# Arsham-001/tsu-emulator

Measured on AMD Instinct MI355X. Metric: spin-updates/sec on L×L 2D Ising Gibbs sweep; achieved HBM GB/s vs peak, higher is better.
Workload: dtype int8

## Files before the change

### tsu-emulator_amd/csrc/ising2d_tiled.hip

```cpp
#include "ising2d.h"

#include <type_traits>
#include <vector>

typedef short v2s __attribute__((ext_vector_type(2)));
typedef unsigned short v2us __attribute__((ext_vector_type(2)));

struct TiledParams {
    const int8_t* src;
    int8_t* dst;
    long long pitch;
    int rows, nchunks;
    int cols;
    int q_shift;
    int tile_h;
    int flex_ty;
    int r_begin, r_end;
    long long row0, total_rows;
    int wrap_rows, ghost;
    int k;
    int tiles_x;
    int ty_first, ty_stride;
    uint32_t k0, k1, sweep0, tag_hi, tag_lo;
    uint32_t tblH0, tblH1, tblL0, tblL1;
    uint32_t t3H0, t3H1, t3L0, t3L1;
    int open;
    uint64_t thr[25];
};

static __host__ __device__ __forceinline__ void tile_rows(const TiledParams& p, int ty, int& row_off, int& H) {
    H = p.tile_h;
    row_off = ty * p.tile_h;
    if (p.flex_ty > 0) {
        const long long half = (p.r_end - p.r_begin + 1) / 2;
        row_off = 2 * (int)(ty * half / p.flex_ty);
        H = 2 * (int)((ty + 1) * half / p.flex_ty) - row_off;
    }
}
static __host__ __device__ __forceinline__ bool tile_holds_wrap(const TiledParams& p, int ty, int k, long long& rg0) {
    int H, row_off;
    tile_rows(p, ty, row_off, H);
    rg0 = p.row0 + p.r_begin + row_off - 2 * k;
    if (p.open) return false;
    rg0 %= p.total_rows;
    if (rg0 < 0) rg0 += p.total_rows;
    return rg0 + H + 4 * k > p.total_rows;
}
static __host__ __device__ __forceinline__ bool wrap_by_mask(const TiledParams& p) { return (p.total_rows & (p.total_rows - 1)) == 0; }

static __device__ __forceinline__ uint32_t perm(uint32_t s0, uint32_t s1, uint32_t sel) {
    return __builtin_amdgcn_perm(s0, s1, sel);
}
static __device__ __forceinline__ uint32_t subsat16(uint32_t a, uint32_t b) {
    return __builtin_bit_cast(uint32_t, __builtin_elementwise_sub_sat(__builtin_bit_cast(v2s, a), __builtin_bit_cast(v2s, b)));
}
static __device__ __forceinline__ uint32_t minu16(uint32_t a, uint32_t b) {
    return __builtin_bit_cast(uint32_t, __builtin_elementwise_min(__builtin_bit_cast(v2us, a), __builtin_bit_cast(v2us, b)));
}

static __device__ __noinline__ u32x4 resolve_ties(u32x4 d, u32x4 w, uint32_t cnt_lo, uint32_t cnt_hi, const uint64_t* s_thr,
                                                  uint32_t cq, uint32_t Rg, uint32_t hs, uint32_t tag_lo, uint32_t k0,
                                                  uint32_t k1, uint32_t edge = 0) {
    const u32x4 l = tsu_philox(cq, Rg, hs, tag_lo, k0, k1);
#define TSU_FIX(DW, WW, LW, CNT, B0, M0)                                                                        \
    _Pragma("unroll") for (int hlf = 0; hlf < 2; ++hlf) {                                                       \
        const uint32_t sh = 16u * hlf;                                                                          \
        if (((DW >> sh) & 0xFFFFu) == 0) {                                                                      \
            const uint32_t c = (CNT >> (8 * (B0 + hlf))) & 0xFFu;                                               \
            const uint32_t m = M0 + hlf;                                                                        \
            const uint32_t deg = 4u - (edge & 1u) - ((m == 0 && (edge & 2u)) ? 1u : 0u) - ((m == (edge >> 4) && (edge & 4u)) ? 1u : 0u); \
            const uint64_t u = ((uint64_t)(((WW >> sh) & 0xFFFFu) ^ 0x8000u) << 16) | ((LW >> sh) & 0xFFFFu);   \
            const uint32_t f = (u < s_thr[deg * 5 + c]) ? 0x8000u : 0x0001u;       \
            DW = (DW & ~(0xFFFFu << sh)) | (f << sh);                                                           \
        }                                                                                                       \
    }
    TSU_FIX(d.x, w.x, l.x, cnt_lo, 0, 0)
    TSU_FIX(d.y, w.y, l.y, cnt_lo, 2, 2)
    TSU_FIX(d.z, w.z, l.z, cnt_hi, 0, 4)
    TSU_FIX(d.w, w.w, l.w, cnt_hi, 2, 6)
#undef TSU_FIX
    return d;
}

struct PhiloxKeys {
    uint32_t a[10], b[10];
};

static __device__ __forceinline__ PhiloxKeys make_keys(uint32_t k0, uint32_t k1) {
    PhiloxKeys K;
#pragma unroll
    for (int r = 0; r < 10; ++r) {
        uint32_t x = k0 + (uint32_t)r * TSU_PHILOX_W0, y = k1 + (uint32_t)r * TSU_PHILOX_W1;
        if (r > 0) asm volatile("v_mov_b32 %0, %1" : "=v"(x) : "s"(x));
        asm volatile("v_mov_b32 %0, %1" : "=v"(y) : "s"(y));
        K.a[r] = x;
        K.b[r] = y;
    }
    return K;
}

static __device__ __forceinline__ uint32_t and_xor(uint32_t a, uint32_t b, uint32_t c) { return __builtin_amdgcn_bitop3_b32(a, b, c, 0x6A); }

static __device__ __forceinline__ uint32_t philox_y0(uint32_t hs, uint32_t k0) {
    uint32_t y = (uint32_t)(((uint64_t)TSU_PHILOX_M1 * hs) >> 32) ^ k0;
    asm volatile("v_mov_b32 %0, %1" : "=v"(y) : "s"(y));
    return y;
}

static __device__ __forceinline__ u32x4 philox_vk(uint32_t c0, uint32_t row, uint32_t rmask, uint32_t y0, uint32_t c2, uint32_t c3,
                                                  const PhiloxKeys& K) {
    uint32_t c1;
    {
        const uint64_t p0 = (uint64_t)TSU_PHILOX_M0 * c0;
        const uint64_t p1 = (uint64_t)TSU_PHILOX_M1 * c2;
        const uint32_t n0 = and_xor(row, rmask, y0);
        const uint32_t n2 = tsu_xor3((uint32_t)(p0 >> 32), c3, K.b[0]);
        c1 = (uint32_t)p1;
        c3 = (uint32_t)p0;
        c0 = n0;
        c2 = n2;
    }
#pragma unroll
    for (int r = 1; r < 10; ++r) {
        uint64_t p0 = (uint64_t)TSU_PHILOX_M0 * c0;
        uint64_t p1 = (uint64_t)TSU_PHILOX_M1 * c2;
        uint32_t n0 = tsu_xor3((uint32_t)(p1 >> 32), c1, K.a[r]);
        uint32_t n2 = tsu_xor3((uint32_t)(p0 >> 32), c3, K.b[r]);
        c1 = (uint32_t)p1;
        c3 = (uint32_t)p0;
        c0 = n0;
        c2 = n2;
    }
    return u32x4{c0, c1, c2, c3};
}

struct Rows2Ctx {
    const uint64_t* s_thr;
    int total_rows;
    int rg_tile0, wrap_tr;
    uint32_t rmask;
    uint32_t tag_hi, tag_lo, k0, k1;
    uint32_t tblH0, tblH1, tblL0, tblL1;
    uint32_t t3H0, t3H1, t3L0, t3L1;
    int last_row;
    bool lft, rgt;
    uint32_t r_par, r_slot;
    uint32_t rm_lo, rm_hi;
    uint64_t vm_e, vm_o;
    uint32_t nvm_e, nvm_o;
    int sh_next, sh_prev;
};

static __device__ __forceinline__ u32x4 compare_octet(const u32x4& w, uint32_t cnt_lo, uint32_t cnt_hi, uint32_t tH0,
                                                      uint32_t tH1, uint32_t tL0, uint32_t tL1) {
    const uint32_t Hl = perm(tH1, tH0, cnt_lo), Ll = perm(tL1, tL0, cnt_lo);
    const uint32_t Hh = perm(tH1, tH0, cnt_hi), Lh = perm(tL1, tL0, cnt_hi);
    u32x4 d;
    d.x = subsat16(w.x, perm(Hl, Ll, 0x05010400u));
    d.y = subsat16(w.y, perm(Hl, Ll, 0x07030602u));
    d.z = subsat16(w.z, perm(Hh, Lh, 0x05010400u));
    d.w = subsat16(w.w, perm(Hh, Lh, 0x07030602u));
    return d;
}

static __device__ __forceinline__ u32x4 compare_octet_open(const u32x4& w, uint32_t cnt_lo, uint32_t cnt_hi, const Rows2Ctx& c,
                                                           bool row_edge, bool l0, bool r7) {
    uint32_t Hl = perm(c.tblH1, c.tblH0, cnt_lo), Ll = perm(c.tblL1, c.tblL0, cnt_lo);
    uint32_t Hh = perm(c.tblH1, c.tblH0, cnt_hi), Lh = perm(c.tblL1, c.tblL0, cnt_hi);
    if (row_edge | l0 | r7) {
        const uint32_t rl = r7 ? c.rm_lo : 0u, rh = r7 ? c.rm_hi : 0u;
        const uint32_t il = cnt_lo + ((row_edge && l0) ? 0x00000004u : 0u) + (row_edge ? (rl & 0x04040404u) : 0u);
        const uint32_t ih = cnt_hi + (row_edge ? (rh & 0x04040404u) : 0u);
        const uint32_t ml = row_edge ? 0xFFFFFFFFu : ((l0 ? 0x000000FFu : 0u) | rl), mh = row_edge ? 0xFFFFFFFFu : rh;
        Hl = (Hl & ~ml) | (perm(c.t3H1, c.t3H0, il) & ml);
        Ll = (Ll & ~ml) | (perm(c.t3L1, c.t3L0, il) & ml);
        Hh = (Hh & ~mh) | (perm(c.t3H1, c.t3H0, ih) & mh);
        Lh = (Lh & ~mh) | (perm(c.t3L1, c.t3L0, ih) & mh);
    }
    u32x4 d;
    d.x = subsat16(w.x, perm(Hl, Ll, 0x05010400u));
    d.y = subsat16(w.y, perm(Hl, Ll, 0x07030602u));
    d.z = subsat16(w.z, perm(Hh, Lh, 0x05010400u));
    d.w = subsat16(w.w, perm(Hh, Lh, 0x07030602u));
    return d;
}

static __device__ __forceinline__ bool has_zero_field(const u32x4& d) {
    const uint32_t mn = minu16(minu16(d.x, d.y), minu16(d.z, d.w));
    return ((mn & 0xFFFFu) == 0) | ((mn >> 16) == 0);
}

static __device__ __forceinline__ uint64_t pack_flags(const u32x4& d) {
    const uint32_t nlo = perm(d.y, d.x, 0x0B0A0908u) & 0x01010101u;
    const uint32_t nhi = perm(d.w, d.z, 0x0B0A0908u) & 0x01010101u;
    return (uint64_t)nlo | ((uint64_t)nhi << 32);
}

template <int NO>
static __device__ __forceinline__ void edge_rows(const Rows2Ctx& c, int to_wrap, int tr, int& rga, int& rgb) {
    constexpr int SPAN = 2 * ((NO - 1 + 63) / NO) + 1;
    const int s_off = to_wrap > 0 ? c.rg_tile0 : c.rg_tile0 - c.total_rows;
    rga = tr + s_off;
    rgb = rga + 1;
    if (__builtin_expect((uint32_t)(to_wrap - 1) < (uint32_t)SPAN, 0)) {
        rga = tr + c.rg_tile0;
        asm volatile("" : "+v"(rga));
        rgb = rga + 1;
        if (rga >= c.total_rows) rga -= c.total_rows;
        if (rgb >= c.total_rows) rgb -= c.total_rows;
    }
}

#define TSU_LDS __attribute__((address_space(3)))
static __device__ __forceinline__ uint32_t lds_addr(const void* p) { return (uint32_t)(uintptr_t)(const TSU_LDS char*)p; }
template <typename T>
static __device__ __forceinline__ T lds_ld(uint32_t a) { return *(const TSU_LDS T*)(uintptr_t)a; }
template <typename T>
static __device__ __forceinline__ void lds_st(uint32_t a, T v) { *(TSU_LDS T*)(uintptr_t)a = v; }

template <typename E, int NO>
struct TilePlanes {
    E* base;
// ... 17 lines not shown
    const u32x4 w0 = philox_vk(cq, (uint32_t)rga, c.rmask, y0, hs, c.tag_hi, K);
    const u32x4 w1 = philox_vk(cq, (uint32_t)rgb, c.rmask, y0, hs, c.tag_hi, K);
    __builtin_amdgcn_sched_barrier(0);
    const uint32_t C0l = (uint32_t)R1, C0h = (uint32_t)(R1 >> 32), C1l = (uint32_t)R2, C1h = (uint32_t)(R2 >> 32);
    uint32_t S0l = P0 ? __builtin_amdgcn_alignbyte(C0h, C0l, 1) : __builtin_amdgcn_alignbyte(C0l, A0, 3);
    uint32_t S0h = P0 ? __builtin_amdgcn_alignbyte(A0, C0h, 1) : __builtin_amdgcn_alignbyte(C0h, C0l, 3);
    uint32_t S1l = P0 ? __builtin_amdgcn_alignbyte(C1l, A1, 3) : __builtin_amdgcn_alignbyte(C1h, C1l, 1);
    uint32_t S1h = P0 ? __builtin_amdgcn_alignbyte(C1h, C1l, 3) : __builtin_amdgcn_alignbyte(A1, C1h, 1);
    if (SEAM) {
        const uint64_t nxa = (Na & 0xFFull) << c.sh_next, pva = (Na >> c.sh_prev) & 0xFFull;
        const uint64_t nxb = (Nb & 0xFFull) << c.sh_next, pvb = (Nb >> c.sh_prev) & 0xFFull;
        const uint64_t Sa = P0 ? ((R1 >> 8) | nxa) : ((R1 << 8) | pva);
        const uint64_t Sb = P0 ? ((R2 << 8) | pvb) : ((R2 >> 8) | nxb);
        S0l = (uint32_t)Sa; S0h = (uint32_t)(Sa >> 32);
        S1l = (uint32_t)Sb; S1h = (uint32_t)(Sb >> 32);
    }
    const uint32_t ml = C0l + C1l, mh = C0h + C1h;
    const uint32_t cnt0l = (uint32_t)R0 + ml + S0l, cnt0h = (uint32_t)(R0 >> 32) + mh + S0h;
    const uint32_t cnt1l = (uint32_t)R3 + ml + S1l, cnt1h = (uint32_t)(R3 >> 32) + mh + S1h;
    u32x4 d0, d1;
    uint32_t edge_a = 0, edge_b = 0;
    if (OPEN) {
        const bool ea = rga == 0 || rga == c.last_row, eb = rgb == 0 || rgb == c.last_row;
        const bool la = !P0 && c.lft, ra = c.rgt && c.r_par == (uint32_t)P0, lb = P0 && c.lft, rb = c.rgt && c.r_par != (uint32_t)P0;
        d0 = compare_octet_open(w0, cnt0l, cnt0h, c, ea, la, ra);
        d1 = compare_octet_open(w1, cnt1l, cnt1h, c, eb, lb, rb);
        edge_a = (ea ? 1u : 0u) | (la ? 2u : 0u) | (ra ? 4u : 0u) | (c.r_slot << 4);
        edge_b = (eb ? 1u : 0u) | (lb ? 2u : 0u) | (rb ? 4u : 0u) | (c.r_slot << 4);
    } else {
        d0 = compare_octet(w0, cnt0l, cnt0h, c.tblH0, c.tblH1, c.tblL0, c.tblL1);
        d1 = compare_octet(w1, cnt1l, cnt1h, c.tblH0, c.tblH1, c.tblL0, c.tblL1);
    }
    const uint32_t mn = minu16(minu16(minu16(d0.x, d0.y), minu16(d0.z, d0.w)), minu16(minu16(d1.x, d1.y), minu16(d1.z, d1.w)));
    if (__builtin_expect(((mn & 0xFFFFu) == 0) | ((mn >> 16) == 0), 0)) {
        if (has_zero_field(d0)) d0 = resolve_ties(d0, w0, cnt0l, cnt0h, c.s_thr, cq, (uint32_t)rga & c.rmask, hs, c.tag_lo, c.k0, c.k1, edge_a);
        if (has_zero_field(d1)) d1 = resolve_ties(d1, w1, cnt1l, cnt1h, c.s_thr, cq, (uint32_t)rgb & c.rmask, hs, c.tag_lo, c.k0, c.k1, edge_b);
    }
    uint64_t n0 = pack_flags(d0), n1 = pack_flags(d1);
    if (OPEN) {
        n0 = (rga < 0 || rga > c.last_row) ? 0 : (n0 & (P0 ? c.vm_o : c.vm_e));
        n1 = (rgb < 0 || rgb > c.last_row) ? 0 : (n1 & (P0 ? c.vm_e : c.vm_o));
    }
    if (SEAM) {
        n0 &= c.vm_e;
        n1 &= c.vm_e;
    }
    lds_st<uint64_t>(a + RS + DO, n0);
    lds_st<uint64_t>(a + 2 * RS + DO, n1);
}

template <int NO, int RL, int KAPPA, int P0, bool EDGE, bool OPEN, bool SEAM = false>
static __device__ __forceinline__ void sweep_pairs(const Rows2Ctx& c, const PhiloxKeys& K, uint32_t hs, uint32_t y0, uint32_t a, int rg, int n, bool tail,
                                                   uint32_t cq) {
    int to_wrap = EDGE ? c.wrap_tr - __builtin_amdgcn_readfirstlane(rg) : 0;
    bool live = true;
#pragma unroll 1
    for (int i = n; i >= 0; --i) {
        if (i == 0) live = tail;
        asm volatile("" : "+v"(a), "+v"(rg));
        if (live) pair_step<NO, KAPPA, P0, EDGE, OPEN, SEAM>(c, K, hs, y0, a, rg, to_wrap, cq);
        a += 2 * RL * 2 * NO * 8;
        rg += 2 * RL;
        to_wrap -= 2 * RL;
    }
}


static __device__ __forceinline__ uint32_t nib_shift_next(uint32_t X, uint32_t N) {
    const uint32_t hi = (N << 4) | __builtin_amdgcn_ubfe(X, 4u, 4u);
// ... 22 lines not shown
    constexpr int DO = (KAPPA ? NO : -NO) * 4;
    const uint32_t R0 = lds_ld<uint32_t>(a), R1 = lds_ld<uint32_t>(a + RS);
    const uint32_t R2 = lds_ld<uint32_t>(a + 2 * RS), R3 = lds_ld<uint32_t>(a + 3 * RS);
    const uint32_t A0 = lds_ld<uint32_t>(a + RS + (P0 ? 4 : -4));
    const uint32_t A1 = lds_ld<uint32_t>(a + 2 * RS + (P0 ? -4 : 4));
    __builtin_amdgcn_sched_barrier(0);
    int rga = rg, rgb = rg + 1;
    if (EDGE) edge_rows<NO>(c, to_wrap, rg, rga, rgb);
    const u32x4 w0 = philox_vk(cq, (uint32_t)rga, c.rmask, y0, hs, c.tag_hi, K);
    const u32x4 w1 = philox_vk(cq, (uint32_t)rgb, c.rmask, y0, hs, c.tag_hi, K);
    __builtin_amdgcn_sched_barrier(0);
    const uint32_t Sa = SEAM ? (P0 ? nib_shift_next_seam(R1, A0, c.sh_next) : nib_shift_prev_seam(R1, A0, c.sh_prev))
                             : (P0 ? nib_shift_next(R1, A0) : nib_shift_prev(R1, A0));
    const uint32_t Sb = SEAM ? (P0 ? nib_shift_prev_seam(R2, A1, c.sh_prev) : nib_shift_next_seam(R2, A1, c.sh_next))
                             : (P0 ? nib_shift_prev(R2, A1) : nib_shift_next(R2, A1));
    const uint32_t mid = R1 + R2;
    const uint32_t cnt0 = R0 + mid + Sa, cnt1 = R3 + mid + Sb;
    const uint32_t cnt0l = cnt0 & 0x0F0F0F0Fu, cnt0h = (cnt0 >> 4) & 0x0F0F0F0Fu;
    const uint32_t cnt1l = cnt1 & 0x0F0F0F0Fu, cnt1h = (cnt1 >> 4) & 0x0F0F0F0Fu;
    u32x4 d0, d1;
    uint32_t edge_a = 0, edge_b = 0;
    if (OPEN) {
        const bool ea = rga == 0 || rga == c.last_row, eb = rgb == 0 || rgb == c.last_row;
        const bool la = !P0 && c.lft, ra = c.rgt && c.r_par == (uint32_t)P0, lb = P0 && c.lft, rb = c.rgt && c.r_par != (uint32_t)P0;
        d0 = compare_octet_open(w0, cnt0l, cnt0h, c, ea, la, ra);
        d1 = compare_octet_open(w1, cnt1l, cnt1h, c, eb, lb, rb);
        edge_a = (ea ? 1u : 0u) | (la ? 2u : 0u) | (ra ? 4u : 0u) | (c.r_slot << 4);
        edge_b = (eb ? 1u : 0u) | (lb ? 2u : 0u) | (rb ? 4u : 0u) | (c.r_slot << 4);
    } else {
        d0 = compare_octet(w0, cnt0l, cnt0h, c.tblH0, c.tblH1, c.tblL0, c.tblL1);
        d1 = compare_octet(w1, cnt1l, cnt1h, c.tblH0, c.tblH1, c.tblL0, c.tblL1);
    }
    const uint32_t mn = minu16(minu16(minu16(d0.x, d0.y), minu16(d0.z, d0.w)), minu16(minu16(d1.x, d1.y), minu16(d1.z, d1.w)));
    if (__builtin_expect(((mn & 0xFFFFu) == 0) | ((mn >> 16) == 0), 0)) {
        if (has_zero_field(d0)) d0 = resolve_ties(d0, w0, cnt0l, cnt0h, c.s_thr, cq, (uint32_t)rga & c.rmask, hs, c.tag_lo, c.k0, c.k1, edge_a);
        if (has_zero_field(d1)) d1 = resolve_ties(d1, w1, cnt1l, cnt1h, c.s_thr, cq, (uint32_t)rgb & c.rmask, hs, c.tag_lo, c.k0, c.k1, edge_b);
    }
    uint32_t n0 = nib_pack(d0), n1 = nib_pack(d1);
    if (OPEN) {
        n0 = (rga < 0 || rga > c.last_row) ? 0u : (n0 & (P0 ? c.nvm_o : c.nvm_e));
        n1 = (rgb < 0 || rgb > c.last_row) ? 0u : (n1 & (P0 ? c.nvm_e : c.nvm_o));
    }
    if (SEAM) {
        n0 &= c.nvm_e;
        n1 &= c.nvm_e;
    }
    lds_st<uint32_t>(a + RS + DO, n0);
    lds_st<uint32_t>(a + 2 * RS + DO, n1);
}

template <int NO, int RL, int KAPPA, int P0, bool EDGE, bool OPEN = false, bool SEAM = false>
static __device__ __forceinline__ void sweep_pairs_nib(const Rows2Ctx& c, const PhiloxKeys& K, uint32_t hs, uint32_t y0, uint32_t a, int rg, int n, bool tail,
                                                       uint32_t cq) {
    int to_wrap = EDGE ? c.wrap_tr - __builtin_amdgcn_readfirstlane(rg) : 0;
    bool live = true;
#pragma unroll 1
    for (int i = n; i >= 0; --i) {
        if (i == 0) live = tail;
        asm volatile("" : "+v"(a), "+v"(rg));
        if (live) pair_step_nib<NO, KAPPA, P0, EDGE, OPEN, SEAM>(c, K, hs, y0, a, rg, to_wrap, cq);
        a += 2 * RL * 2 * NO * 4;
        rg += 2 * RL;
        to_wrap -= 2 * RL;
    }
}

template <int NO, int RL, int KAPPA, int P0, bool EDGE, bool OPEN, bool SEAM, bool NIB>
static __device__ __forceinline__ void half_sweep(const Rows2Ctx& c, const PhiloxKeys& K, int TR, uint32_t sweep, int s, uint32_t a_thr, int al,
                                                  uint32_t cq) {
// ... 25 lines not shown
                                                        int al, uint32_t cq) {
#pragma unroll 1
    for (int s = 0; s < kg; ++s) {
        half_sweep<NO, RL, 0, P0, EDGE, OPEN, SEAM, NIB>(c, K, TR, sweep_g + (uint32_t)s, s, a_thr, al, cq);
        half_sweep<NO, RL, 1, P0, EDGE, OPEN, SEAM, NIB>(c, K, TR, sweep_g + (uint32_t)s, s, a_thr, al, cq);
    }
}

static __device__ __forceinline__ void xst(uint64_t* p, uint64_t v) { __hip_atomic_store(p, v, __ATOMIC_RELAXED, __HIP_MEMORY_SCOPE_AGENT); }
static __device__ __forceinline__ uint64_t xld(const uint64_t* p) { return __hip_atomic_load(p, __ATOMIC_RELAXED, __HIP_MEMORY_SCOPE_AGENT); }

struct ResidentParams {
    uint64_t* xbuf;
    uint32_t gen0;
    int* err;
    int n_gen, k_last, tiles_y;
    int wrap_y;
    int wrap_x;
    long long* dbg;
};

template <int HT, int WO, int THREADS, bool OPEN = false, bool RESIDENT = false, bool NIB = false>
static __device__ __forceinline__ void tile_body(const TiledParams& p, const int8_t* __restrict__ src, int8_t* __restrict__ dst,
                                                 const int k, const uint32_t sweep0, const int tx, const int ty, uint64_t* lds,
                                                 const PhiloxKeys& K, const ResidentParams* R = nullptr) {
    constexpr int NO = WO + 2;
    constexpr int RLMAX = THREADS / NO;
    int H, row_off;
    tile_rows(p, ty, row_off, H);
    const int TR = H + 4 * k;
    constexpr int RL = RLMAX;
    using E = typename std::conditional<NIB, uint32_t, uint64_t>::type;
    const TilePlanes<E, NO> P{reinterpret_cast<E*>(lds + 1)};
    uint64_t* s_thr = reinterpret_cast<uint64_t*>((reinterpret_cast<uintptr_t>(P.base + 2 * TR * NO + NO + 1) + 7u) & ~(uintptr_t)7u);
    const int tid = threadIdx.x;
    if (tid < 25) s_thr[tid] = p.thr[tid];

    const int q0 = tx * WO + p.q_shift, r0 = p.r_begin + row_off, Rb = r0 - 2 * k;

    const int al = tid / NO, oct = tid - al * NO;
    int cqi = q0 - 1 + oct;
    const bool col_out = OPEN && (cqi < 0 || cqi >= p.nchunks);
    if (!OPEN) {
        if (cqi < 0) cqi += p.nchunks;
        if (cqi >= p.nchunks) cqi -= p.nchunks;
        if (cqi >= p.nchunks) cqi -= p.nchunks;
    }
    const uint32_t cq = (uint32_t)cqi;
    int nv = p.cols - 16 * cqi;
    if (col_out) nv = 0;
    if (nv > 16) nv = 16;
    auto first_sites = [](int n) { return n >= 8 ? 0x0101010101010101ull : (((1ull << (8 * n)) - 1) & 0x0101010101010101ull); };
    const uint64_t vm_e = first_sites((nv + 1) >> 1), vm_o = first_sites(nv >> 1);

    if (al < RLMAX) {
        const int8_t* col = src + 16 * (long long)(OPEN ? (cqi < 0 ? 0 : (cqi >= p.nchunks ? p.nchunks - 1 : cqi)) : cqi);
        constexpr int LB = 4;
        for (int tr0 = al; tr0 < TR; tr0 += LB * RLMAX) {
            uint4 v[LB];
#pragma unroll
            for (int b = 0; b < LB; ++b) {
                const int tr = tr0 + b * RLMAX;
                const int rl = Rb + (tr < TR ? tr : TR - 1);
                int srow;
                if (p.wrap_rows) srow = rl < 0 ? rl + p.rows : (rl >= p.rows ? rl - p.rows : rl);
                else srow = rl < -p.ghost ? -p.ghost : (rl >= p.rows + p.ghost ? p.rows + p.ghost - 1 : rl);
                v[b] = *reinterpret_cast<const uint4*>(col + (long long)srow * p.pitch);
            }
#pragma unroll
            for (int b = 0; b < LB; ++b) {
                const int tr = tr0 + b * RLMAX;
                if (tr < TR) {
                    const uint32_t e0 = perm(v[b].y, v[b].x, 0x06040200u), e1 = perm(v[b].w, v[b].z, 0x06040200u);
                    const uint32_t o0 = perm(v[b].y, v[b].x, 0x07050301u), o1 = perm(v[b].w, v[b].z, 0x07050301u);
                    uint64_t ev = (uint64_t)(~(e0 >> 1) & 0x01010101u) | ((uint64_t)(~(e1 >> 1) & 0x01010101u) << 32);
                    uint64_t od = (uint64_t)(~(o0 >> 1) & 0x01010101u) | ((uint64_t)(~(o1 >> 1) & 0x01010101u) << 32);
                    if (OPEN) {
                        const long long grow = p.row0 + Rb + tr;
                        if (grow < 0 || grow >= p.total_rows) ev = od = 0;
                    }
                    if (OPEN || nv < 16) {
                        ev &= vm_e;
                        od &= vm_o;
                    }
                    const int gpar = (int)((p.row0 + Rb + tr) & 1);
                    if (NIB) {
                        P.at(gpar, tr, oct) = (E)((uint32_t)ev | ((uint32_t)(ev >> 32) << 4));
                        P.at(gpar ^ 1, tr, oct) = (E)((uint32_t)od | ((uint32_t)(od >> 32) << 4));
                    } else {
                        P.at(gpar, tr, oct) = (E)ev;
                        P.at(gpar ^ 1, tr, oct) = (E)od;
                    }
                }
            }
        }
    }

    long long rg0;
    const bool holds_wrap = tile_holds_wrap(p, ty, k, rg0);
    const bool edge = holds_wrap && !wrap_by_mask(p);

    Rows2Ctx c;
    c.s_thr = s_thr;
    c.total_rows = (int)p.total_rows;
    c.rg_tile0 = (int)rg0;
    c.wrap_tr = (int)(p.total_rows - rg0);
    asm volatile("v_mov_b32 %0, %1" : "=v"(c.rmask) : "s"(holds_wrap && !edge ? (uint32_t)p.total_rows - 1u : 0xFFFFFFFFu));
    c.tag_hi = p.tag_hi; c.tag_lo = p.tag_lo; c.k0 = p.k0; c.k1 = p.k1;
    c.tblH0 = p.tblH0; c.tblH1 = p.tblH1; c.tblL0 = p.tblL0; c.tblL1 = p.tblL1;
    c.t3H0 = p.t3H0; c.t3H1 = p.t3H1; c.t3L0 = p.t3L0; c.t3L1 = p.t3L1;
    c.last_row = (int)p.total_rows - 1;
    c.lft = OPEN && cqi == 0;
    c.rgt = OPEN && cqi == p.nchunks - 1;
    c.r_par = (uint32_t)(p.cols - 1) & 1u;
    c.r_slot = ((uint32_t)(p.cols - 1) & 15u) >> 1;
    c.rm_lo = c.r_slot < 4 ? 0xFFu << (8 * c.r_slot) : 0u;
    c.rm_hi = c.r_slot < 4 ? 0u : 0xFFu << (8 * (c.r_slot - 4));
    c.vm_e = NIB ? 0 : vm_e;
    c.vm_o = NIB ? 0 : vm_o;
    c.nvm_e = NIB ? ((uint32_t)vm_e | ((uint32_t)(vm_e >> 32) << 4)) : 0u;
    c.nvm_o = NIB ? ((uint32_t)vm_o | ((uint32_t)(vm_o >> 32) << 4)) : 0u;
    const int v_last = (p.cols >> 1) & 7;
    const bool ragged = !OPEN && v_last != 0;
    const int seam_site = v_last - 1;
    const int seam_pos = NIB ? 8 * (seam_site & 3) + 4 * (seam_site >> 2) : 8 * seam_site, last_pos = NIB ? 28 : 56;
    c.sh_next = (ragged && cqi == p.nchunks - 1) ? seam_pos : last_pos;
    c.sh_prev = (ragged && cqi == 0) ? seam_pos : last_pos;
    int w0 = (q0 - 1) % p.nchunks;
    if (w0 < 0) w0 += p.nchunks;
    const bool seam = ragged && (w0 == 0 || w0 + NO - 1 >= p.nchunks - 1);
    asm volatile("v_mov_b32 %0, %1" : "=v"(c.tblH0) : "s"(p.tblH0));
    asm volatile("v_mov_b32 %0, %1" : "=v"(c.tblH1) : "s"(p.tblH1));
    asm volatile("v_mov_b32 %0, %1" : "=v"(c.tblL0) : "s"(p.tblL0));
    asm volatile("v_mov_b32 %0, %1" : "=v"(c.tblL1) : "s"(p.tblL1));

    const int n_gen = RESIDENT ? R->n_gen : 1;
// ... 241 lines not shown
    {256, 32, 512, k1_tiled2<256, 32, 512, 4, false, true>, nullptr, k1_tiled2<256, 32, 512, 4, true, true>, nullptr, 1, 2},
};
constexpr int kNumVariants = sizeof(kVariants) / sizeof(kVariants[0]);

int ragged_shift(const tsu_ising2d* L, int WO) {
    if (!L->periodic || L->cols % 16 == 0) return 0;
    const int nch = (L->cols + 15) / 16, tiles_x = (nch + WO - 1) / WO;
    for (int shift = 1; shift < WO && shift < nch - 1; ++shift) {
        bool ok = true;
        for (int t = 0; t < tiles_x && ok; ++t) {
            const int s = t * WO + shift;
            if (s % nch == 0) ok = false;
            if (t < tiles_x - 1 && (s + WO) % nch == nch - 1) ok = false;
        }
        if (ok) return shift;
    }
    return -1;
}

size_t lds_share(const TileVariant& tv) { return (size_t)(160 / tv.per_cu) * 1024; }

int chip_cus(const tsu_ising2d* L) { return L->ctx->cus > 0 ? L->ctx->cus : 256; }

int lattice_env(const char* name, int dflt) {
    const char* e = getenv(name);
    return e ? atoi(e) : dflt;
}

double gen_time_us(const TileVariant& c, int h, double between) {
    const int pairs = (h + 4 * 8 - 2) / 2, waves = (pairs * (c.WO + 2) + 63) / 64;
    return 16.0 * (0.25 + (c.nib ? 1.06 : 1.0) * 0.225 * ((waves + 3) / 4)) + between;
}

template <typename P>
void pack_thresholds(P& p, const uint64_t table[25]) {
    for (int c = 0; c < 25; ++c) p.thr[c] = table[c];
    auto top16 = [](uint64_t thr) {
        uint32_t thi = (uint32_t)(thr >> 16);
        if (thi > 65535u) thi = 65535u;
        return thi ^ 0x8000u;
    };
    uint32_t t16[5], t3[8] = {0, 0, 0, 0, 0, 0, 0, 0};
    for (int c = 0; c < 5; ++c) t16[c] = top16(table[4 * 5 + c]);
    for (int c = 0; c < 4; ++c) t3[c] = top16(table[3 * 5 + c]);
    for (int c = 0; c < 3; ++c) t3[4 + c] = top16(table[2 * 5 + c]);
    p.t3L0 = (t3[0] & 0xFF) | ((t3[1] & 0xFF) << 8) | ((t3[2] & 0xFF) << 16) | ((t3[3] & 0xFF) << 24);
    p.t3L1 = (t3[4] & 0xFF) | ((t3[5] & 0xFF) << 8) | ((t3[6] & 0xFF) << 16);
    p.t3H0 = (t3[0] >> 8) | ((t3[1] >> 8) << 8) | ((t3[2] >> 8) << 16) | ((t3[3] >> 8) << 24);
    p.t3H1 = (t3[4] >> 8) | ((t3[5] >> 8) << 8) | ((t3[6] >> 8) << 16);
    p.tblL0 = (t16[0] & 0xFF) | ((t16[1] & 0xFF) << 8) | ((t16[2] & 0xFF) << 16) | ((t16[3] & 0xFF) << 24);
    p.tblL1 = (t16[4] & 0xFF);
    p.tblH0 = (t16[0] >> 8) | ((t16[1] >> 8) << 8) | ((t16[2] >> 8) << 16) | ((t16[3] >> 8) << 24);
    p.tblH1 = (t16[4] >> 8);
}

int flex_cut(const tsu_ising2d* L, int v, int* v_out, int* hmax_out, double* t_out) {
    if (L->ghost != 0 || L->total_rows != L->rows) return 0;
    if (L->periodic && ((L->cols & 1) || (L->rows & 1))) return 0;
    const int FLEX_HMIN = 16;
    static const int max_tiles = lattice_env("TSU_K1_FLEX_MAX_TILES", 0);
    int cus = chip_cus(L);
    if (max_tiles > 0 && max_tiles < cus) cus = max_tiles;
    const int nch = (L->cols + 15) / 16;
    static const int cand[] = {V_256x512_T1024, V_128x256_T1024, V_N512x512_T1024};
    double best = 1e300;
    int best_ty = 0;
    for (int ci = 0; ci < (int)(sizeof(cand) / sizeof(cand[0])); ++ci) {
        if (v >= 0 && cand[ci] != v) continue;
        const TileVariant& c = kVariants[cand[ci]];
// ... 218 lines not shown
        p.src = L->alloc[L->cur] + (size_t)L->ghost * L->pitch;
        p.dst = L->alloc[L->cur ^ 1] + (size_t)L->ghost * L->pitch;
        p.tile_h = c.tile_h;
        p.flex_ty = c.flex_ty;
        p.r_begin = -c.res_ext;
        p.r_end = L->rows + c.res_ext;
        P.t = p;
        P.r.wrap_y = L->wrap_rows ? 1 : 0;
        P.r.wrap_x = L->periodic ? 1 : 0;
        P.r.xbuf = L->d_xbuf;
        const bool renumber = L->xsig != xsig || L->xgen + (uint32_t)((chunk + kmax - 1) / kmax) + 2u >= 16383u;
        if (renumber) {
            L->xsig = xsig;
            L->xgen = 0;
        }
        P.r.gen0 = L->xgen + 1u;
        L->xgen += (uint32_t)((chunk + kmax - 1) / kmax);
        P.r.err = d_err;
        P.r.n_gen = (chunk + kmax - 1) / kmax;
        P.r.k_last = chunk - (P.r.n_gen - 1) * kmax;
        P.r.tiles_y = c.tiles_y;
        P.r.dbg = nullptr;
        long long* d_dbg = nullptr;
        if (verbose >= 2) {
            TSU_HIP_TRY(ctx, hipMalloc(&d_dbg, (size_t)4 * ntiles * sizeof(long long)));
            P.r.dbg = d_dbg;
        }
        if (verbose) {
            bool any_wrap = false;
            for (int ty = 0; ty < c.tiles_y && !any_wrap; ++ty) {
                long long rg0;
                any_wrap = tile_holds_wrap(P.t, ty, kmax, rg0);
            }
            fprintf(stderr, "[tsu] k1_resident variant %d: %d tiles (%d per CU fit), %d generations of %d sweeps, %zu KB of strips, row wrap: %s\n",
                    c.v, ntiles, fit_per_cu, P.r.n_gen, kmax, xneed * 8 / 1024, !any_wrap ? "none" : (wrap_by_mask(P.t) ? "mask" : "compare"));
        }
        {
            const int rcx = tsu_grid_exclusive_begin(ctx);
            if (rcx != TSU_OK) return rcx;
        }
        if (renumber) TSU_HIP_TRY(ctx, hipMemsetAsync(L->d_xbuf, 0, L->xbuf_cap, ctx->stream));
        TSU_HIP_TRY(ctx, tsu_launch_grid_sync(ctx, (const void*)res_kern, dim3((unsigned)ntiles), dim3((unsigned)tv.threads), &P, lds_bytes, ctx->stream,
                                              !whole));
        L->launches += 1;
        L->cur ^= 1;
        {
            const int rcx = tsu_grid_exclusive_end(ctx);
            if (rcx != TSU_OK) return rcx;
        }
        if (d_dbg) {
            print_resident_timeline(d_dbg, ntiles, p.tiles_x, c.tiles_y, P.r.n_gen, verbose);
            (void)hipFree(d_dbg);
        }
        done += chunk;
    }
    return TSU_OK;
}

int run_generations(tsu_ising2d* L, const CallPlan& c, TiledParams p, int n_sweeps, uint32_t sweep0, int part) {
    tsu_ctx* ctx = L->ctx;
    const TileVariant& tv = kVariants[c.v];
    void (*const kern)(TiledParams) = L->periodic ? tv.kernel : tv.open;
    const bool slab = !(L->wrap_rows || (!L->periodic && L->ghost == 0 && L->total_rows == L->rows));
    for (int done = 0; done < n_sweeps;) {
        const int k = n_sweeps - done < c.kmax ? n_sweeps - done : c.kmax;
        p.k = k;
        p.sweep0 = sweep0 + (uint32_t)done;
        p.src = L->alloc[L->cur] + (size_t)L->ghost * L->pitch;
// ... 62 lines not shown
    p.cols = L->cols;
    p.row0 = L->row0;
    p.total_rows = L->total_rows;
    p.wrap_rows = L->wrap_rows;
    p.ghost = L->ghost;
    p.tiles_x = (p.nchunks + tv.WO - 1) / tv.WO;
    p.q_shift = ragged_shift(L, tv.WO);
    p.r_begin = 0;
    p.r_end = L->rows;
    p.tile_h = tv.H;
    p.flex_ty = 0;
    ising2d_set_keys(p, seed, replica);
    pack_thresholds(p, L->table);
    p.open = L->periodic ? 0 : 1;
    TSU_HIP_TRY(ctx, tsu_func_allow_lds(ctx, (const void*)(L->periodic ? tv.kernel : tv.open), 160 * 1024));
    if (c.resident) {
        void (*const res_kern)(ResidentLaunch) = L->periodic ? tv.resident : tv.resident_open;
        TSU_HIP_TRY(ctx, tsu_func_allow_lds(ctx, (const void*)res_kern, 160 * 1024));
        int fit_per_cu = 0;
        TSU_HIP_TRY(ctx, tsu_func_blocks_per_cu(ctx, (const void*)res_kern, tv.threads, tile_lds_bytes(tv, (c.flex_ty > 0 ? c.tile_h : tv.H) + 4 * KMAX),
                                                &fit_per_cu));
        if ((long long)p.tiles_x * c.tiles_y <= (long long)fit_per_cu * ctx->cus) return run_resident(L, c, p, n_sweeps, sweep0, fit_per_cu);
    }
    return run_generations(L, c, p, n_sweeps, sweep0, part);
}

struct PlanesItem {
    int8_t* buf;
    long long pitch;
    int rows, cols, periodic;
    uint32_t k0, k1, tag_hi, tag_lo, sweep0;
    uint32_t tblH0, tblH1, tblL0, tblL1, t3H0, t3H1, t3L0, t3L1;
    uint64_t thr[25];
};

template <bool OPEN>
__global__ __launch_bounds__(1024) void k1_planes(const PlanesItem* __restrict__ items, PlanesItem one, int n_sweeps) {
    __shared__ uint64_t s_planes[2 * 1024];
    __shared__ uint64_t s_thr[25];
    const PlanesItem& it = items ? items[blockIdx.x] : one;
    const int tid = threadIdx.x;
    const int rows = it.rows, cols = it.cols, nch = (cols + 15) >> 4, tasks = rows * nch;
    if (tid < 25) s_thr[tid] = it.thr[tid];
    const PhiloxKeys K = make_keys(it.k0, it.k1);
    const bool active = tid < tasks;
    const int r = active ? tid / nch : 0, q = active ? tid - r * nch : 0;
    const int idx = r * nch + q;
    uint64_t* const plane0 = s_planes;
    uint64_t* const plane1 = s_planes + tasks;
    int nv = cols - 16 * q;
    if (nv > 16) nv = 16;
    auto first_sites = [](int n) { return n >= 8 ? 0x0101010101010101ull : (((1ull << (8 * n)) - 1) & 0x0101010101010101ull); };
    const uint64_t vm_e = first_sites((nv + 1) >> 1), vm_o = first_sites(nv >> 1);
    int8_t* const chunk = it.buf + (long long)r * it.pitch + 16 * q;
    if (active) {
        const uint4 v = *reinterpret_cast<const uint4*>(chunk);
        const uint32_t e0 = perm(v.y, v.x, 0x06040200u), e1 = perm(v.w, v.z, 0x06040200u);
        const uint32_t o0 = perm(v.y, v.x, 0x07050301u), o1 = perm(v.w, v.z, 0x07050301u);
        uint64_t ev = (uint64_t)(~(e0 >> 1) & 0x01010101u) | ((uint64_t)(~(e1 >> 1) & 0x01010101u) << 32);
        uint64_t od = (uint64_t)(~(o0 >> 1) & 0x01010101u) | ((uint64_t)(~(o1 >> 1) & 0x01010101u) << 32);
        ev &= vm_e;
        od &= vm_o;
        ((r & 1) ? plane1 : plane0)[idx] = ev;
        ((r & 1) ? plane0 : plane1)[idx] = od;
    }
    const int up = r > 0 ? idx - nch : (OPEN ? -1 : idx + (rows - 1) * nch);
    const int dn = r < rows - 1 ? idx + nch : (OPEN ? -1 : idx - (rows - 1) * nch);
    const int lf = q > 0 ? idx - 1 : (OPEN ? -1 : idx + nch - 1);
    const int rt = q < nch - 1 ? idx + 1 : (OPEN ? -1 : idx - (nch - 1));
    const int v_last = ((cols >> 1) & 7) ? ((cols >> 1) & 7) : 8;
    const int shl = q == nch - 1 ? 8 * (v_last - 1) : 56, shr = q == 0 ? 8 * (v_last - 1) : 56;
    Rows2Ctx c;
    c.s_thr = s_thr;
    c.t3H0 = it.t3H0; c.t3H1 = it.t3H1; c.t3L0 = it.t3L0; c.t3L1 = it.t3L1;
    asm volatile("v_mov_b32 %0, %1" : "=v"(c.tblH0) : "s"(it.tblH0));
    asm volatile("v_mov_b32 %0, %1" : "=v"(c.tblH1) : "s"(it.tblH1));
    asm volatile("v_mov_b32 %0, %1" : "=v"(c.tblL0) : "s"(it.tblL0));
    asm volatile("v_mov_b32 %0, %1" : "=v"(c.tblL1) : "s"(it.tblL1));
    c.r_par = (uint32_t)(cols - 1) & 1u;
    c.r_slot = ((uint32_t)(cols - 1) & 15u) >> 1;
    c.rm_lo = c.r_slot < 4 ? 0xFFu << (8 * c.r_slot) : 0u;
    c.rm_hi = c.r_slot < 4 ? 0u : 0xFFu << (8 * (c.r_slot - 4));
    const bool row_edge = OPEN && (r == 0 || r == rows - 1);
    const uint32_t tag_hi = it.tag_hi, tag_lo = it.tag_lo, k0 = it.k0, k1 = it.k1, sweep0 = it.sweep0;
    for (int hsi = 0; hsi < 2 * n_sweeps; ++hsi) {
        __syncthreads();
        const int kappa = hsi & 1;
        const uint32_t hs = 2u * (sweep0 + (uint32_t)(hsi >> 1)) + (uint32_t)kappa;
        if (active) {
            const uint64_t* Ps = kappa ? plane0 : plane1;
            uint64_t* Pd = kappa ? plane1 : plane0;
            const int par = (r + kappa) & 1;
            const uint64_t U = (OPEN && up < 0) ? 0ull : Ps[up], D = (OPEN && dn < 0) ? 0ull : Ps[dn], C = Ps[idx];
            const int side = par ? rt : lf;
            const uint64_t A = (OPEN && side < 0) ? 0ull : Ps[side];
            const uint64_t S = par ? ((C >> 8) | ((A & 0xFFull) << shl)) : ((C << 8) | ((A >> shr) & 0xFFull));
            const uint64_t cnt = U + D + C + S;
            const uint32_t cnt_lo = (uint32_t)cnt, cnt_hi = (uint32_t)(cnt >> 32);
            const u32x4 w = philox_vk((uint32_t)q, (uint32_t)r, 0xFFFFFFFFu, philox_y0(hs, k0), hs, tag_hi, K);
            u32x4 d;
            uint32_t edge = 0;
            if (OPEN) {
                const bool l0 = !par && q == 0, r7 = q == nch - 1 && c.r_par == (uint32_t)par;
                d = compare_octet_open(w, cnt_lo, cnt_hi, c, row_edge, l0, r7);
                edge = (row_edge ? 1u : 0u) | (l0 ? 2u : 0u) | (r7 ? 4u : 0u) | (c.r_slot << 4);
            } else {
                d = compare_octet(w, cnt_lo, cnt_hi, c.tblH0, c.tblH1, c.tblL0, c.tblL1);
            }
            if (__builtin_expect(has_zero_field(d), 0)) d = resolve_ties(d, w, cnt_lo, cnt_hi, s_thr, (uint32_t)q, (uint32_t)r, hs, tag_lo, k0, k1, edge);
            uint64_t n = pack_flags(d);
            n &= par ? vm_o : vm_e;
            Pd[idx] = n;
        }
    }
    __syncthreads();
    if (active) {
        const uint64_t ev = ((r & 1) ? plane1 : plane0)[idx], od = ((r & 1) ? plane0 : plane1)[idx];
        const uint32_t e0 = perm(0u, 0x000001FFu, (uint32_t)ev), e1 = perm(0u, 0x000001FFu, (uint32_t)(ev >> 32));
        const uint32_t o0 = perm(0u, 0x000001FFu, (uint32_t)od), o1 = perm(0u, 0x000001FFu, (uint32_t)(od >> 32));
        uint4 v = make_uint4(perm(o0, e0, 0x05010400u), perm(o0, e0, 0x07030602u), perm(o1, e1, 0x05010400u), perm(o1, e1, 0x07030602u));
        if (nv < 16) {
            auto bytes = [](int n) { return n >= 4 ? 0xFFFFFFFFu : (n <= 0 ? 0u : (1u << (8 * n)) - 1u); };
            v.x &= bytes(nv);
            v.y &= bytes(nv - 4);
            v.z &= bytes(nv - 8);
            v.w &= bytes(nv - 12);
        }
        *reinterpret_cast<uint4*>(chunk) = v;
    }
}

int tsu_ising2d_planes_supported(const tsu_ising2d* L) {
    if (L->ghost != 0 || L->total_rows != L->rows || L->row0 != 0) return 0;
    if ((long long)L->rows * ((L->cols + 15) / 16) > 1024) return 0;
    return L->rows >= 2 && L->cols >= 2;
}

int tsu_ising2d_planes_sweep(tsu_ising2d* const* lats, int n, int n_sweeps, const uint64_t* seeds, const uint32_t* sweep0s,
                             const uint32_t* replicas) {
    tsu_ctx* ctx = lats[0]->ctx;
    std::vector<PlanesItem> items((size_t)n);
    for (int i = 0; i < n; ++i) {
// ... 30 lines not shown
```

Before: 3206 billion.

## Scalarize tie resolution per lane and read threshold table from kernargs

Rewrites the rare tie-resolution path so it walks the active lanes one at a time, running Philox and the threshold lookup with scalar registers and scalar loads from the kernel-argument segment instead of a shared-memory copy. This drops the per-block LDS staging of the 25-entry threshold table along with its store. It also adds a configurable tie window, default 1, so the fast-path compare can flag near-ties as well as exact ones. The cost is a serial per-lane loop when ties occur, plus a dependence on the kernarg layout that static_asserts guard.

Result: slower. 3173 billion (-1.0%).

```diff
diff --git a/tsu-emulator_amd/csrc/ising2d_tiled.hip b/tsu-emulator_amd/csrc/ising2d_tiled.hip
--- a/tsu-emulator_amd/csrc/ising2d_tiled.hip
+++ b/tsu-emulator_amd/csrc/ising2d_tiled.hip
@@ -1,5 +1,6 @@
 #include "ising2d.h"
 
+#include <cstddef>
 #include <type_traits>
 #include <vector>
 
@@ -26,6 +27,7 @@
     uint32_t t3H0, t3H1, t3L0, t3L1;
     int open;
     uint64_t thr[25];
+    uint64_t tie_window;
 };
 
 static __host__ __device__ __forceinline__ void tile_rows(const TiledParams& p, int ty, int& row_off, int& H) {
@@ -58,27 +60,81 @@
     return __builtin_bit_cast(uint32_t, __builtin_elementwise_min(__builtin_bit_cast(v2us, a), __builtin_bit_cast(v2us, b)));
 }
 
+typedef const uint64_t __attribute__((address_space(4))) * tie_table_ptr;
+struct TieTable {
+    uint64_t thr[25];
+    uint64_t tie_window;
+};
+
+static __device__ __forceinline__ const uint64_t* kernarg_tie_table(size_t offset) {
+    return (const uint64_t*)((const __attribute__((address_space(4))) char*)__builtin_amdgcn_kernarg_segment_ptr() + offset);
+}
+
+static __device__ __forceinline__ u32x4 philox_uniform(uint32_t c0, uint32_t c1, uint32_t c2, uint32_t c3, uint32_t k0, uint32_t k1) {
+#pragma unroll
+    for (int r = 0; r < 10; ++r) {
+        const uint64_t p0 = (uint64_t)TSU_PHILOX_M0 * c0;
+        const uint64_t p1 = (uint64_t)TSU_PHILOX_M1 * c2;
+        const uint32_t n0 = (uint32_t)(p1 >> 32) ^ c1 ^ k0;
+        const uint32_t n2 = (uint32_t)(p0 >> 32) ^ c3 ^ k1;
+        c1 = (uint32_t)p1;
+        c3 = (uint32_t)p0;
+        c0 = n0;
+        c2 = n2;
+        k0 += TSU_PHILOX_W0;
+        k1 += TSU_PHILOX_W1;
+    }
+    return u32x4{c0, c1, c2, c3};
+}
+
 static __device__ __noinline__ u32x4 resolve_ties(u32x4 d, u32x4 w, uint32_t cnt_lo, uint32_t cnt_hi, const uint64_t* s_thr,
                                                   uint32_t cq, uint32_t Rg, uint32_t hs, uint32_t tag_lo, uint32_t k0,
                                                   uint32_t k1, uint32_t edge = 0) {
-    const u32x4 l = tsu_philox(cq, Rg, hs, tag_lo, k0, k1);
+    const uint32_t u_hs = __builtin_amdgcn_readfirstlane(hs), u_tag = __builtin_amdgcn_readfirstlane(tag_lo);
+    const uint32_t u_k0 = __builtin_amdgcn_readfirstlane(k0), u_k1 = __builtin_amdgcn_readfirstlane(k1);
+    const uint64_t tp = (uint64_t)(uintptr_t)s_thr;
+    const uint32_t tp_lo = (uint32_t)__builtin_amdgcn_readfirstlane((uint32_t)tp), tp_hi = (uint32_t)__builtin_amdgcn_readfirstlane((uint32_t)(tp >> 32));
+    const tie_table_ptr thr = (tie_table_ptr)(uintptr_t)(((uint64_t)tp_hi << 32) | tp_lo);
+    const uint32_t win = (uint32_t)thr[25];
+    const uint32_t me = __lane_id();
+    for (uint64_t todo = __ballot(1); todo != 0; todo &= todo - 1) {
+        const int lane = __builtin_ctzll(todo);
+        uint32_t dx = __builtin_amdgcn_readlane(d.x, lane), dy = __builtin_amdgcn_readlane(d.y, lane);
+        uint32_t dz = __builtin_amdgcn_readlane(d.z, lane), dw = __builtin_amdgcn_readlane(d.w, lane);
+        const uint32_t wx = __builtin_amdgcn_readlane(w.x, lane), wy = __builtin_amdgcn_readlane(w.y, lane);
+        const uint32_t wz = __builtin_amdgcn_readlane(w.z, lane), ww = __builtin_amdgcn_readlane(w.w, lane);
+        const uint32_t c_lo = __builtin_amdgcn_readlane(cnt_lo, lane), c_hi = __builtin_amdgcn_readlane(cnt_hi, lane);
+        const uint32_t e = __builtin_amdgcn_readlane(edge, lane);
+        uint32_t e_k0 = u_k0, e_k1 = u_k1;
+        asm volatile("" : "+s"(e_k0), "+s"(e_k1));
+        const u32x4 l = philox_uniform(__builtin_amdgcn_readlane(cq, lane), __builtin_amdgcn_readlane(Rg, lane), u_hs, u_tag, e_k0, e_k1);
 #define TSU_FIX(DW, WW, LW, CNT, B0, M0)                                                                        \
     _Pragma("unroll") for (int hlf = 0; hlf < 2; ++hlf) {                                                       \
         const uint32_t sh = 16u * hlf;                                                                          \
-        if (((DW >> sh) & 0xFFFFu) == 0) {                                                                      \
+        if (((DW >> sh) & 0xFFFFu) < win) {                                                                     \
             const uint32_t c = (CNT >> (8 * (B0 + hlf))) & 0xFFu;                                               \
             const uint32_t m = M0 + hlf;                                                                        \
-            const uint32_t deg = 4u - (edge & 1u) - ((m == 0 && (edge & 2u)) ? 1u : 0u) - ((m == (edge >> 4) && (edge & 4u)) ? 1u : 0u); \
-            const uint64_t u = ((uint64_t)(((WW >> sh) & 0xFFFFu) ^ 0x8000u) << 16) | ((LW >> sh) & 0xFFFFu);   \
-            const uint32_t f = (u < s_thr[deg * 5 + c]) ? 0x8000u : 0x0001u;       \
+            const uint32_t deg = 4u - (e & 1u) - (m == 0 ? (e >> 1) & 1u : 0u) - (m == (e >> 4) ? (e >> 2) & 1u : 0u); \
+            const uint32_t ti = deg * 5 + c;  \
+            const uint32_t u = ((((WW >> sh) & 0xFFFFu) ^ 0x8000u) << 16) | ((LW >> sh) & 0xFFFFu);             \
+            const uint64_t t = thr[ti < 24u ? ti : 24u];                         \
+            uint32_t t_hi = (uint32_t)(t >> 32);                                                                \
+            asm("" : "+s"(t_hi));  \
+            const uint32_t f = (t_hi != 0 || u < (uint32_t)t) ? 0x8000u : 0x0001u;  \
             DW = (DW & ~(0xFFFFu << sh)) | (f << sh);                                                           \
         }                                                                                                       \
     }
-    TSU_FIX(d.x, w.x, l.x, cnt_lo, 0, 0)
-    TSU_FIX(d.y, w.y, l.y, cnt_lo, 2, 2)
-    TSU_FIX(d.z, w.z, l.z, cnt_hi, 0, 4)
-    TSU_FIX(d.w, w.w, l.w, cnt_hi, 2, 6)
+        TSU_FIX(dx, wx, l.x, c_lo, 0, 0)
+        TSU_FIX(dy, wy, l.y, c_lo, 2, 2)
+        TSU_FIX(dz, wz, l.z, c_hi, 0, 4)
+        TSU_FIX(dw, ww, l.w, c_hi, 2, 6)
 #undef TSU_FIX
+        const bool mine = me == (uint32_t)lane;
+        d.x = mine ? dx : d.x;
+        d.y = mine ? dy : d.y;
+        d.z = mine ? dz : d.z;
+        d.w = mine ? dw : d.w;
+    }
     return d;
 }
 
@@ -136,6 +192,7 @@
 
 struct Rows2Ctx {
     const uint64_t* s_thr;
+    uint32_t win, win_hi;
     int total_rows;
     int rg_tile0, wrap_tr;
     uint32_t rmask;
@@ -185,9 +242,9 @@
     return d;
 }
 
-static __device__ __forceinline__ bool has_zero_field(const u32x4& d) {
-    const uint32_t mn = minu16(minu16(d.x, d.y), minu16(d.z, d.w));
-    return ((mn & 0xFFFFu) == 0) | ((mn >> 16) == 0);
+static __device__ __forceinline__ bool min_is_tied(uint32_t mn, uint32_t win, uint32_t win_hi) { return ((mn & 0xFFFFu) < win) | (mn < win_hi); }
+static __device__ __forceinline__ bool has_tied_field(const u32x4& d, uint32_t win, uint32_t win_hi) {
+    return min_is_tied(minu16(minu16(d.x, d.y), minu16(d.z, d.w)), win, win_hi);
 }
 
 static __device__ __forceinline__ uint64_t pack_flags(const u32x4& d) {
@@ -271,9 +328,9 @@
         d1 = compare_octet(w1, cnt1l, cnt1h, c.tblH0, c.tblH1, c.tblL0, c.tblL1);
     }
     const uint32_t mn = minu16(minu16(minu16(d0.x, d0.y), minu16(d0.z, d0.w)), minu16(minu16(d1.x, d1.y), minu16(d1.z, d1.w)));
-    if (__builtin_expect(((mn & 0xFFFFu) == 0) | ((mn >> 16) == 0), 0)) {
-        if (has_zero_field(d0)) d0 = resolve_ties(d0, w0, cnt0l, cnt0h, c.s_thr, cq, (uint32_t)rga & c.rmask, hs, c.tag_lo, c.k0, c.k1, edge_a);
-        if (has_zero_field(d1)) d1 = resolve_ties(d1, w1, cnt1l, cnt1h, c.s_thr, cq, (uint32_t)rgb & c.rmask, hs, c.tag_lo, c.k0, c.k1, edge_b);
+    if (__builtin_expect(min_is_tied(mn, c.win, c.win_hi), 0)) {
+        if (has_tied_field(d0, c.win, c.win_hi)) d0 = resolve_ties(d0, w0, cnt0l, cnt0h, c.s_thr, cq, (uint32_t)rga & c.rmask, hs, c.tag_lo, c.k0, c.k1, edge_a);
+        if (has_tied_field(d1, c.win, c.win_hi)) d1 = resolve_ties(d1, w1, cnt1l, cnt1h, c.s_thr, cq, (uint32_t)rgb & c.rmask, hs, c.tag_lo, c.k0, c.k1, edge_b);
     }
     uint64_t n0 = pack_flags(d0), n1 = pack_flags(d1);
     if (OPEN) {
@@ -362,9 +419,9 @@
         d1 = compare_octet(w1, cnt1l, cnt1h, c.tblH0, c.tblH1, c.tblL0, c.tblL1);
     }
     const uint32_t mn = minu16(minu16(minu16(d0.x, d0.y), minu16(d0.z, d0.w)), minu16(minu16(d1.x, d1.y), minu16(d1.z, d1.w)));
-    if (__builtin_expect(((mn & 0xFFFFu) == 0) | ((mn >> 16) == 0), 0)) {
-        if (has_zero_field(d0)) d0 = resolve_ties(d0, w0, cnt0l, cnt0h, c.s_thr, cq, (uint32_t)rga & c.rmask, hs, c.tag_lo, c.k0, c.k1, edge_a);
-        if (has_zero_field(d1)) d1 = resolve_ties(d1, w1, cnt1l, cnt1h, c.s_thr, cq, (uint32_t)rgb & c.rmask, hs, c.tag_lo, c.k0, c.k1, edge_b);
+    if (__builtin_expect(min_is_tied(mn, c.win, c.win_hi), 0)) {
+        if (has_tied_field(d0, c.win, c.win_hi)) d0 = resolve_ties(d0, w0, cnt0l, cnt0h, c.s_thr, cq, (uint32_t)rga & c.rmask, hs, c.tag_lo, c.k0, c.k1, edge_a);
+        if (has_tied_field(d1, c.win, c.win_hi)) d1 = resolve_ties(d1, w1, cnt1l, cnt1h, c.s_thr, cq, (uint32_t)rgb & c.rmask, hs, c.tag_lo, c.k0, c.k1, edge_b);
     }
     uint32_t n0 = nib_pack(d0), n1 = nib_pack(d1);
     if (OPEN) {
@@ -456,9 +513,7 @@
     constexpr int RL = RLMAX;
     using E = typename std::conditional<NIB, uint32_t, uint64_t>::type;
     const TilePlanes<E, NO> P{reinterpret_cast<E*>(lds + 1)};
-    uint64_t* s_thr = reinterpret_cast<uint64_t*>((reinterpret_cast<uintptr_t>(P.base + 2 * TR * NO + NO + 1) + 7u) & ~(uintptr_t)7u);
     const int tid = threadIdx.x;
-    if (tid < 25) s_thr[tid] = p.thr[tid];
 
     const int q0 = tx * WO + p.q_shift, r0 = p.r_begin + row_off, Rb = r0 - 2 * k;
 
@@ -525,7 +580,10 @@
     const bool edge = holds_wrap && !wrap_by_mask(p);
 
     Rows2Ctx c;
-    c.s_thr = s_thr;
+    static_assert(offsetof(TiledParams, tie_window) == offsetof(TiledParams, thr) + offsetof(TieTable, tie_window), "TieTable layout");
+    c.s_thr = kernarg_tie_table(offsetof(TiledParams, thr));
+    c.win = (uint32_t)p.tie_window;
+    c.win_hi = c.win << 16;
     c.total_rows = (int)p.total_rows;
     c.rg_tile0 = (int)rg0;
     c.wrap_tr = (int)(p.total_rows - rg0);
@@ -833,9 +891,15 @@
     return 16.0 * (0.25 + (c.nib ? 1.06 : 1.0) * 0.225 * ((waves + 3) / 4)) + between;
 }
 
+uint64_t tie_window() {
+    static const int env = lattice_env("TSU_K1_TIE_WINDOW", 1);
+    return (uint64_t)(env < 1 ? 1 : (env > 0x8000 ? 0x8000 : env));
+}
+
 template <typename P>
 void pack_thresholds(P& p, const uint64_t table[25]) {
     for (int c = 0; c < 25; ++c) p.thr[c] = table[c];
+    p.tie_window = tie_window();
     auto top16 = [](uint64_t thr) {
         uint32_t thi = (uint32_t)(thr >> 16);
         if (thi > 65535u) thi = 65535u;
@@ -1120,8 +1184,8 @@
                 long long rg0;
                 any_wrap = tile_holds_wrap(P.t, ty, kmax, rg0);
             }
-            fprintf(stderr, "[tsu] k1_resident variant %d: %d tiles (%d per CU fit), %d generations of %d sweeps, %zu KB of strips, row wrap: %s\n",
-                    c.v, ntiles, fit_per_cu, P.r.n_gen, kmax, xneed * 8 / 1024, !any_wrap ? "none" : (wrap_by_mask(P.t) ? "mask" : "compare"));
+            fprintf(stderr, "[tsu] k1_resident variant %d: %d tiles (%d per CU fit), %d generations of %d sweeps, %zu KB of strips, tie window %d, row wrap: %s\n",
+                    c.v, ntiles, fit_per_cu, P.r.n_gen, kmax, xneed * 8 / 1024, (int)P.t.tie_window, !any_wrap ? "none" : (wrap_by_mask(P.t) ? "mask" : "compare"));
         }
         {
             const int rcx = tsu_grid_exclusive_begin(ctx);
@@ -1250,16 +1314,17 @@
     uint32_t k0, k1, tag_hi, tag_lo, sweep0;
     uint32_t tblH0, tblH1, tblL0, tblL1, t3H0, t3H1, t3L0, t3L1;
     uint64_t thr[25];
+    uint64_t tie_window;
 };
 
 template <bool OPEN>
 __global__ __launch_bounds__(1024) void k1_planes(const PlanesItem* __restrict__ items, PlanesItem one, int n_sweeps) {
     __shared__ uint64_t s_planes[2 * 1024];
-    __shared__ uint64_t s_thr[25];
     const PlanesItem& it = items ? items[blockIdx.x] : one;
+    static_assert(offsetof(PlanesItem, tie_window) == offsetof(PlanesItem, thr) + offsetof(TieTable, tie_window) && alignof(PlanesItem) == 8, "TieTable layout");
+    const uint64_t* const s_thr = items ? items[blockIdx.x].thr : kernarg_tie_table(8 + offsetof(PlanesItem, thr));
     const int tid = threadIdx.x;
     const int rows = it.rows, cols = it.cols, nch = (cols + 15) >> 4, tasks = rows * nch;
-    if (tid < 25) s_thr[tid] = it.thr[tid];
     const PhiloxKeys K = make_keys(it.k0, it.k1);
     const bool active = tid < tasks;
     const int r = active ? tid / nch : 0, q = active ? tid - r * nch : 0;
@@ -1290,6 +1355,8 @@
     const int shl = q == nch - 1 ? 8 * (v_last - 1) : 56, shr = q == 0 ? 8 * (v_last - 1) : 56;
     Rows2Ctx c;
     c.s_thr = s_thr;
+    c.win = (uint32_t)it.tie_window;
+    c.win_hi = c.win << 16;
     c.t3H0 = it.t3H0; c.t3H1 = it.t3H1; c.t3L0 = it.t3L0; c.t3L1 = it.t3L1;
     asm volatile("v_mov_b32 %0, %1" : "=v"(c.tblH0) : "s"(it.tblH0));
     asm volatile("v_mov_b32 %0, %1" : "=v"(c.tblH1) : "s"(it.tblH1));
@@ -1325,7 +1392,7 @@
             } else {
                 d = compare_octet(w, cnt_lo, cnt_hi, c.tblH0, c.tblH1, c.tblL0, c.tblL1);
             }
-            if (__builtin_expect(has_zero_field(d), 0)) d = resolve_ties(d, w, cnt_lo, cnt_hi, s_thr, (uint32_t)q, (uint32_t)r, hs, tag_lo, k0, k1, edge);
+            if (__builtin_expect(has_tied_field(d, c.win, c.win_hi), 0)) d = resolve_ties(d, w, cnt_lo, cnt_hi, s_thr, (uint32_t)q, (uint32_t)r, hs, tag_lo, k0, k1, edge);
             uint64_t n = pack_flags(d);
             n &= par ? vm_o : vm_e;
             Pd[idx] = n;
```
